# tangjiapeng/DiffuScene

Measured on AMD Instinct MI355X. Metric: denoiser steps/sec (train + 1000-step sample) at B=256, N=80 objects, higher is better.
Workload: dtype f32 (operands split 3xbf16, 6 products, f32 accumulate); 1 GPU; uncond living/dining rooms (config/uncond/diffusion_livingrooms_instancond_lat32_v.yaml scaled to N=80), B=256 scenes per GPU, N=80, C=65, T=1000, mode=both; global_batch=256, parallelism=single

## Files before the change

### diffuscene_amd/_lib.py

```python
import ctypes as C
import os

_HERE = os.path.dirname(os.path.abspath(__file__))
LIB_PATH = os.path.join(_HERE, "libdiffuscene_hip.so")
if os.environ.get("DSC_HIP_LIB"):
    LIB_PATH = os.path.abspath(os.environ["DSC_HIP_LIB"])

ACT_NONE, ACT_GELU, ACT_SILU, ACT_LEAKY01 = 0, 1, 2, 3
SS_NONE, SS_PER_TOKEN, SS_PER_SCENE, SS_PER_SLOT, SS_BY_INDEX = 0, 1, 2, 3, 4
MEAN_EPS, MEAN_X0, MEAN_V = 0, 1, 2
TILE_GN_80_W8, TILE_GN_80_W4, TILE_160x256, TILE_160x128_W4 = 1, 2, 5, 8
TILE_WAVE_GN, TILE_WAVE_DENSE, TILE_WAVE_GN_64 = 10, 11, 12
F32_TILE_160x256, F32_TILE_160x128, F32_TILE_128x128, F32_TILE_96x128, F32_TILE_64x64 = 0, 1, 2, 3, 4
DSC_PLANES_NONE = -100
GEMM_ROW_INVARIANT = 1
WS_MAX = 64
MAX_TOKENS_PER_SCENE = 160
STATS_MAX_OBJECTS, STATS_ONE_WAVE_MAX = 160, 32

_ERR = {-1: "DSC_EINVAL (bad shape / null pointer)", -2: "DSC_EALIGN (16-byte alignment required)",
        -3: "DSC_ERANGE (size outside kernel limits)"}

c_f32p = C.c_void_p
c_i64p = C.c_void_p
# ... 118 lines not shown
    "dsc_gather_max_bwd_f32": (C.c_int, [c_f32p, C.c_int64, C.c_void_p, C.c_void_p, C.c_int32, C.c_int32, C.c_int32, c_f32p,
                                         C.c_int64, C.c_void_p]),
    "dsc_bn_workspace_floats": (C.c_int64, [C.c_int64, C.c_int32]),
    "dsc_batchnorm_fwd_f32": (C.c_int, [c_f32p, C.c_int64, c_f32p, c_f32p, C.c_int64, C.c_int32, C.c_float, C.c_float,
                                        C.c_int32, c_f32p, c_f32p, c_f32p, c_f32p, c_f32p, c_f32p, c_f32p, C.c_int64,
                                        C.c_void_p]),
    "dsc_batchnorm_eval_f32": (C.c_int, [c_f32p, C.c_int64, c_f32p, c_f32p, c_f32p, c_f32p, C.c_int64, C.c_int32, C.c_int32,
                                         c_f32p, C.c_void_p]),
    "dsc_batchnorm_bwd_f32": (C.c_int, [c_f32p, c_f32p, c_f32p, c_f32p, c_f32p, C.c_int64, C.c_int32, C.c_int32, c_f32p,
                                        c_f32p, c_f32p, c_f32p, C.c_int64, C.c_void_p]),
    "dsc_rowmax_f32": (C.c_int, [c_f32p, C.c_int64, C.c_int32, C.c_int32, C.c_int32, c_f32p, C.c_void_p, C.c_void_p]),
    "dsc_rowmax_bwd_f32": (C.c_int, [c_f32p, C.c_void_p, C.c_int32, C.c_int32, C.c_int32, c_f32p, C.c_void_p]),
    "dsc_point_affine_f32": (C.c_int, [c_f32p, C.c_int64, C.c_int32, c_f32p, C.c_int64, c_f32p, C.c_int32, C.c_int32,
                                       C.c_int32, C.c_int32, c_f32p, C.c_void_p]),
    "dsc_point_affine_bwd_f32": (C.c_int, [c_f32p, c_f32p, C.c_int64, C.c_int32, c_f32p, C.c_int64, C.c_int32, C.c_int32,
                                           C.c_int32, C.c_int32, c_f32p, C.c_int64, c_f32p, C.c_int64, c_f32p, c_f32p,
                                           C.c_int64, C.c_void_p]),
    "dsc_postfilter_compact_f32": (C.c_int, [c_f32p, C.c_int32, C.c_int32, C.c_int32, C.c_int32, C.c_int32, C.c_int32, c_f32p,
                                             C.c_void_p, C.c_void_p]),
    "dsc_gemm_tn_f32": (C.c_int, [c_f32p, C.c_int64, C.c_int32, c_f32p, C.c_int64, C.c_int32, c_f32p, C.c_int64, c_f32p,
                                  C.c_int64, c_f32p, C.c_int32, C.c_int32, C.c_int32, c_f32p, C.c_int64, C.c_void_p]),
    "dsc_gemm_tn_workspace_floats": (C.c_int64, [C.c_int32, C.c_int32, C.c_int32]),
    "dsc_gemm_tn_grouped_f32": (C.c_int, [C.c_void_p, C.c_int32, C.c_int32, C.c_int32, c_f32p, C.c_int64, C.c_int64,
                                          C.c_void_p]),
    "dsc_gemm_tn_grouped_split_f32": (C.c_int, [C.c_void_p, C.c_int32, C.c_int32, C.c_void_p, C.c_int32, C.c_int32, c_f32p, C.c_int64,
                                                C.c_int64, C.c_int32, C.c_void_p]),
    "dsc_set_tn_split_form": (C.c_int, [C.c_int32]),
    "dsc_get_tn_split_form": (C.c_int, []),
    "dsc_colsum_f32": (C.c_int, [c_f32p, C.c_int64, C.c_int32, C.c_int32, c_f32p, c_f32p, C.c_int64, C.c_void_p]),
    "dsc_colsum_grouped_f32": (C.c_int, [C.c_void_p, C.c_int32, C.c_int32, C.c_void_p]),
    "dsc_gn_silu_bwd_f32": (C.c_int, [c_f32p, C.c_int64, c_f32p, C.c_int64, c_f32p, c_f32p, c_f32p, C.c_int64, C.c_int32,
                                      c_f32p, C.c_int64, c_f32p, c_f32p, c_f32p, C.c_int64, c_f32p, C.c_int64, C.c_int32,
                                      C.c_int32, C.c_int32, C.c_float, C.c_void_p]),
    "dsc_weight_standardize_bwd_f32": (C.c_int, [C.POINTER(WsBwdItem), C.c_int32, C.c_float, C.c_void_p]),
    "dsc_layernorm_bwd_f32": (C.c_int, [c_f32p, C.c_int64, c_f32p, c_f32p, C.c_int64, c_f32p, C.c_int64, c_f32p, C.c_int64, c_f32p,
                                        C.c_int32, C.c_int32, C.c_int32, C.c_float, C.c_void_p]),
    "dsc_linear_attention_bwd_f32": (C.c_int, [c_f32p, C.c_int64] * 7 + [C.c_int32, C.c_int32, C.c_int32, C.c_float,
                                                                          C.c_void_p]),
    "dsc_attention_bwd_f32": (C.c_int, [c_f32p, C.c_int64] * 7 + [C.c_int32, C.c_int32, C.c_float, C.c_void_p]),
    "dsc_retrieve_nearest_f32": (C.c_int, [c_f32p, C.c_void_p, C.c_void_p, c_f32p, C.c_void_p, C.c_void_p, C.c_int32,
                                           C.c_int32, C.c_int32, C.c_void_p, c_f32p, C.c_void_p]),
    "dsc_box_bounds_f32": (C.c_int, [c_f32p, c_f32p, c_f32p, C.c_void_p, C.c_int32, C.c_int32, c_f32p, C.c_void_p]),
    "dsc_scene_stats_f32": (C.c_int, [c_f32p, c_f32p, C.c_void_p, C.c_void_p, C.c_int32, C.c_int32, C.c_int32, C.c_int32,
                                      C.c_void_p, C.c_void_p, C.c_void_p, C.c_void_p, C.c_void_p, C.c_void_p, c_f32p, C.c_void_p]),
    "dsc_encode_scene_batch_f32": (C.c_int, [c_i64p, c_f32p, c_f32p, c_f32p, c_f32p, c_f32p, C.c_int32, C.c_int32, c_i64p,
                                             C.c_void_p, C.c_void_p, C.c_void_p, C.c_int32, C.POINTER(C.c_double), c_f32p,
                                             C.c_int64, c_i64p, C.c_int32, C.c_int32, C.c_void_p]),
    "dsc_chamfer3d_forward_f32": (C.c_int, [c_f32p, c_f32p, c_f32p, c_f32p, C.c_void_p, C.c_void_p, C.c_int32, C.c_int32,
                                            C.c_int32, C.c_void_p]),
    "dsc_chamfer3d_backward_f32": (C.c_int, [c_f32p, c_f32p, c_f32p, c_f32p, C.c_void_p, C.c_void_p, c_f32p, c_f32p,
                                             C.c_int32, C.c_int32, C.c_int32, C.c_void_p]),
    "dsc_grad_sumsq_f32": (C.c_int, [C.c_void_p, C.c_int32, C.c_void_p, C.c_void_p]),
    "dsc_clip_coef_f32": (C.c_int, [C.c_void_p, C.c_int32, C.c_float, c_f32p, c_f32p, C.c_void_p]),
    "dsc_adam_step_f32": (C.c_int, [C.c_void_p, C.c_int32, C.c_float, C.c_float, C.c_float, C.c_float, C.c_float, C.c_float,
                                    c_f32p, C.c_void_p]),
    "dsc_ddpm_loss_f32": (C.c_int, [c_f32p, c_f32p, c_f32p, c_i64p, c_f32p, c_f32p, c_f32p, c_f32p, C.POINTER(C.c_float),
                                    c_f32p, c_f32p, c_f32p] + [C.c_int32] * 12 + [C.c_float, C.c_int32, C.c_void_p]),
    "dsc_copy2d_f32": (C.c_int, [c_f32p, C.c_int64, c_f32p, C.c_int64, C.c_int32, C.c_int32, C.c_void_p]),
    "dsc_add2d_f32": (C.c_int, [c_f32p, C.c_int64, c_f32p, C.c_int64, C.c_int32, C.c_int32, C.c_void_p]),
    "dsc_activation_bwd_f32": (C.c_int, [c_f32p, c_f32p, c_f32p, C.c_int64, C.c_int32, C.c_void_p]),
    "dsc_transpose_batched_f32": (C.c_int, [C.POINTER(WsItem), C.c_int32, C.c_void_p]),
    "dsc_transpose_f32": (C.c_int, [c_f32p, C.c_int64, c_f32p, C.c_int64, C.c_int32, C.c_int32, C.c_void_p]),
    "dsc_complete_overwrite_f32": (C.c_int, [c_f32p, c_f32p, c_f32p, c_i64p, c_f32p, c_f32p, C.c_int32, C.c_int32,
                                             C.c_int32, C.c_int32, C.c_int32, C.c_void_p]),
    "dsc_complete_overwrite_ragged_f32": (C.c_int, [c_f32p, c_f32p, c_f32p, c_i64p, c_i64p, c_f32p, c_f32p, C.c_int32, C.c_int32,
                                                    C.c_int32, C.c_int32, C.c_int32, C.c_void_p]),
# ... 103 lines not shown
```

### diffuscene_amd/csrc/train.hip

```cpp
#define DSC_BAD_INDEX_COUNTER
#include "dsc_common.h"

namespace {

constexpr int TN_BK = 32;
constexpr int TN_LD = 132;

struct TnArgs {
    const float* a1; long lda1; int k1;
    const float* a2; long lda2; int k2;
    const float* dy; long ldd;
    float* out; long ldo;
    float* bias_out;
    long slab;
    long bias_slab;
    int m, n, kvalid;
    int chunk;
    int ktiles;
};

__device__ __forceinline__ void tn_block(const TnArgs& p, const int it, const int jt, const int split, float* As, float* Bs) {
    const int tid = threadIdx.x, lane = tid & 63, wave = tid >> 6;
    const int wi = wave >> 1, wj = wave & 1;
    const int l31 = lane & 31, half = lane >> 5;
    const int i0 = it * 128, j0 = jt * 128;
    const long m_begin = (long)split * p.chunk;
    const long m_end = (m_begin + p.chunk < p.m) ? m_begin + p.chunk : p.m;

    const float* ab;
    long lda;
    int ic;
    int kseg;
    if (i0 < p.k1) { ab = p.a1; lda = p.lda1; ic = i0; kseg = p.k1; }
    else           { ab = p.a2; lda = p.lda2; ic = i0 - p.k1; kseg = p.k2; }
// ... 427 lines not shown
    const int c = blockIdx.x * 64 + (threadIdx.x & 63);
    if (blockIdx.x * 64 >= it.n) return;
    const int rq = threadIdx.x >> 6;
    float s = 0.f;
    if (c < it.n) {
        const float* xp = it.x + (long)rq * it.ldx + c;
        const long step = 4 * it.ldx;
        int r = rq;
        float s0 = 0.f, s1 = 0.f, s2 = 0.f, s3 = 0.f;
        for (; r + 28 < it.m; r += 32, xp += 8 * step) {
            const float v0 = xp[0], v1 = xp[step], v2 = xp[2 * step], v3 = xp[3 * step];
            const float v4 = xp[4 * step], v5 = xp[5 * step], v6 = xp[6 * step], v7 = xp[7 * step];
            s0 += v0; s1 += v1; s2 += v2; s3 += v3;
            s0 += v4; s1 += v5; s2 += v6; s3 += v7;
        }
        for (; r < it.m; r += 4, xp += step) s0 += xp[0];
        s = (s0 + s1) + (s2 + s3);
    }
    red[rq][threadIdx.x & 63] = s;
    __syncthreads();
    if (rq == 0 && c < it.n) it.out[c] = (red[0][threadIdx.x] + red[1][threadIdx.x]) + (red[2][threadIdx.x] + red[3][threadIdx.x]);
}

struct GnBwdArgs {
    const float* z; long ldz;
    const float* dy; long ldy;
    const float* gamma; const float* beta;
    const float* ss; long ld_ss; int ss_mode;
    float* dz; long lddz;
    float* dgamma_p; float* dbeta_p; float* dbias_p;
    long pstride;
    float* dss; long ld_dss;
    int n_tok, C; float eps;
};

__device__ __forceinline__ float block_sum(float v, float* red) {
    v = wave_sum(v);
    __syncthreads();
    if ((threadIdx.x & 63) == 0) red[threadIdx.x >> 6] = v;
    __syncthreads();
    return (red[0] + red[1]) + (red[2] + red[3]);
}

__global__ __launch_bounds__(256) void gn_silu_bwd_kernel(const GnBwdArgs p) {
    extern __shared__ float gnb_cache[];
    __shared__ float red[4];
    __shared__ float csum[5][4][64];
    const int b = blockIdx.x >> 3, g = blockIdx.x & 7;
    const int cl = threadIdx.x & 63, tq = threadIdx.x >> 6;
    const int c = g * 64 + cl;
    const int N = p.n_tok;
    const long tok0 = (long)b * N;
    const float inv_cnt = 1.0f / (64.0f * (float)N);
    float* zc = gnb_cache + cl;
    float* dc = gnb_cache + (long)N * 64 + cl;
    float s = 0.f;
    {
        const float* zp = p.z + (tok0 + tq) * p.ldz + c;
        const float* dp = p.dy + (tok0 + tq) * p.ldy + c;
        const long zs = 4 * p.ldz, ds = 4 * p.ldy;
#pragma unroll 5
        for (int j = tq; j < N; j += 4) {
            const float zv = *zp, dv = *dp;
            zp += zs; dp += ds;
            zc[j * 64] = zv; dc[j * 64] = dv;
            s += zv;
// ... 150 lines not shown
    const float m2 = bsum(S2) * inv_cnt;
#pragma unroll
    for (int i = 0; i < NIT; ++i) {
        const int j = tr + 16 * i;
        if (j < N) {
            f32x4 dzv;
#pragma unroll
            for (int e = 0; e < 4; ++e) { dzv[e] = rs * (dv[i][e] - m1 - zv[i][e] * m2); Gz[e] += dzv[e]; }
            *reinterpret_cast<f32x4*>(p.dz + (tok0 + j) * p.lddz + c) = dzv;
        }
    }
    auto fold = [&](f32x4 v, int slot) {
#pragma unroll
        for (int e = 0; e < 4; ++e) {
            float t = v[e];
            t += __shfl_xor(t, 16, 64);
            t += __shfl_xor(t, 32, 64);
            if ((threadIdx.x & 63) < 16) csum[slot][wave][cq * 4 + e] = t;
        }
    };
    fold(Gg, 0); fold(Gb, 1); fold(Gz, 2); fold(Gsc, 3); fold(Gsh, 4);
    __syncthreads();
    if (threadIdx.x < 64) {
        const int cl = threadIdx.x;
        const long o = (long)b * p.pstride + g * 64 + cl;
        p.dgamma_p[o] = (csum[0][0][cl] + csum[0][1][cl]) + (csum[0][2][cl] + csum[0][3][cl]);
        p.dbeta_p[o] = (csum[1][0][cl] + csum[1][1][cl]) + (csum[1][2][cl] + csum[1][3][cl]);
        p.dbias_p[o] = (csum[2][0][cl] + csum[2][1][cl]) + (csum[2][2][cl] + csum[2][3][cl]);
        if (p.dss && p.ss_mode == DSC_SS_PER_SCENE) {
            p.dss[(long)b * p.ld_dss + g * 64 + cl] = (csum[3][0][cl] + csum[3][1][cl]) + (csum[3][2][cl] + csum[3][3][cl]);
            p.dss[(long)b * p.ld_dss + p.C + g * 64 + cl] = (csum[4][0][cl] + csum[4][1][cl]) + (csum[4][2][cl] + csum[4][3][cl]);
        }
    }
}

struct WsBwdItem { const float* w; const float* dwh; float* dw; int rows; int cols; };
struct WsBwdBatch { WsBwdItem it[DSC_WS_MAX]; };

__global__ __launch_bounds__(256) void ws_bwd_kernel(const WsBwdBatch bch, const float eps) {
    __shared__ float red[4];
    const WsBwdItem it = bch.it[blockIdx.y];
    const int row = blockIdx.x;
    if (row >= it.rows) return;
    const float* w = it.w + (long)row * it.cols;
    const float* g = it.dwh + (long)row * it.cols;
    float* o = it.dw + (long)row * it.cols;
    constexpr int MAXE = 8;
    float v[MAXE], gv[MAXE];
    float s = 0.f;
#pragma unroll
    for (int i = 0; i < MAXE; ++i) {
        const int c = threadIdx.x + 256 * i;
        v[i] = (c < it.cols) ? w[c] : 0.f;
        gv[i] = (c < it.cols) ? g[c] : 0.f;
        s += v[i];
    }
    const float inv = 1.0f / (float)it.cols;
    const float mean = block_sum(s, red) * inv;
    float s2 = 0.f;
#pragma unroll
    for (int i = 0; i < MAXE; ++i) {
        const int c = threadIdx.x + 256 * i;
        const float d = (c < it.cols) ? v[i] - mean : 0.f;
        s2 += d * d;
    }
    const float rs = 1.0f / sqrtf(block_sum(s2, red) * inv + eps);
// ... 675 lines not shown
                                   int64_t partial_stride, float* dss, int64_t ld_dss, int32_t scenes,
                                   int32_t tokens_per_scene, int32_t channels, float eps, dsc_stream_t stream) {
    if (!z || !dy || !gamma || !beta || !dz || !dgamma_p || !dbeta_p || !dbias_p) return DSC_EINVAL;
    if (scenes < 1 || tokens_per_scene < 1 || channels != 512) return DSC_ERANGE;
    if (ss_mode != DSC_SS_NONE && !scale_shift) return DSC_EINVAL;
    GnBwdArgs p{z, (long)ldz, dy, (long)ldy, gamma, beta, ss_mode != DSC_SS_NONE ? scale_shift : nullptr, (long)ld_ss,
                ss_mode, dz, (long)lddz, dgamma_p, dbeta_p, dbias_p, (long)partial_stride, dss, (long)ld_dss, tokens_per_scene,
                channels, eps};
    if (tokens_per_scene > 160) return DSC_ERANGE;
    const size_t lds = (size_t)2 * tokens_per_scene * 64 * sizeof(float);
    DSC_CLEAR_STALE_ERROR();
    const bool v4 = ((ldz | ldy | lddz) & 3) == 0 && dsc_aligned16(z) && dsc_aligned16(dy) && dsc_aligned16(dz) &&
                    dsc_aligned16(gamma) && dsc_aligned16(beta) &&
                    (!p.ss || (dsc_aligned16(p.ss) && (ld_ss & 3) == 0)) &&
                    (!dss || (dsc_aligned16(dss) && (ld_dss & 3) == 0));
    if (lds > 48 * 1024) {
        static bool raised = false;
        if (!raised) {
            hipError_t e = hipFuncSetAttribute(reinterpret_cast<const void*>(gn_silu_bwd_kernel),
                                               hipFuncAttributeMaxDynamicSharedMemorySize, 96 * 1024);
            if (e != hipSuccess) return (int)e;
            raised = true;
        }
    }
    hipStream_t hs = static_cast<hipStream_t>(stream);
    if (v4 && tokens_per_scene <= 32)
        hipLaunchKernelGGL(gn_silu_bwd_reg_kernel<2>, dim3(scenes * 8), dim3(256), 0, hs, p);
    else if (v4 && tokens_per_scene <= 80)
        hipLaunchKernelGGL(gn_silu_bwd_reg_kernel<5>, dim3(scenes * 8), dim3(256), 0, hs, p);
    else if (v4)
        hipLaunchKernelGGL(gn_silu_bwd_reg_kernel<10>, dim3(scenes * 8), dim3(256), 0, hs, p);
    else
        hipLaunchKernelGGL(gn_silu_bwd_kernel, dim3(scenes * 8), dim3(256), lds, static_cast<hipStream_t>(stream), p);
    DSC_LAUNCH_CHECK();
    return 0;
}

extern "C" int dsc_weight_standardize_bwd_f32(const dsc_ws_bwd_item* items, int32_t count, float eps, dsc_stream_t stream) {
    if (!items || count < 1 || count > DSC_WS_MAX) return DSC_EINVAL;
    WsBwdBatch b;
    int maxrows = 0;
    for (int i = 0; i < count; ++i) {
        if (!items[i].w || !items[i].dw_std || !items[i].dw || items[i].rows < 1 || items[i].cols < 1) return DSC_EINVAL;
        if (items[i].cols > 2048) return DSC_ERANGE;
        b.it[i] = WsBwdItem{items[i].w, items[i].dw_std, items[i].dw, items[i].rows, items[i].cols};
        if (items[i].rows > maxrows) maxrows = items[i].rows;
    }
    DSC_CLEAR_STALE_ERROR();
    hipLaunchKernelGGL(ws_bwd_kernel, dim3(maxrows, count), dim3(256), 0, static_cast<hipStream_t>(stream), b, eps);
    DSC_LAUNCH_CHECK();
    return 0;
}

extern "C" int dsc_layernorm_bwd_f32(const float* x, int64_t ldx, const float* g, const float* dy, int64_t ldy, float* dx,
                                     int64_t lddx, const float* addend, int64_t ldadd, float* dg_partial, int32_t partial_rows,
                                     int32_t m, int32_t d, float eps, dsc_stream_t stream) {
    if (!x || !g || !dy || !dx || !dg_partial || m < 1 || partial_rows < 1) return DSC_EINVAL;
    if (d != 512) return DSC_ERANGE;
    if (!dsc_aligned16(x) || !dsc_aligned16(g) || !dsc_aligned16(dy) || !dsc_aligned16(dx) || (ldx & 3) || (ldy & 3) ||
        (lddx & 3) || (addend && (!dsc_aligned16(addend) || (ldadd & 3)))) return DSC_EALIGN;
    DSC_CLEAR_STALE_ERROR();
    hipLaunchKernelGGL(layernorm_bwd_kernel, dim3(partial_rows), dim3(256), 0, static_cast<hipStream_t>(stream),
                       x, (long)ldx, g, dy, (long)ldy, dx, (long)lddx, addend, (long)ldadd, dg_partial, m, eps);
    DSC_LAUNCH_CHECK();
    return 0;
}
// ... 390 lines not shown
```

### diffuscene_amd/ops.py

```python
import ctypes as C
import numbers

import torch

from . import _lib
from ._lib import (ACT_GELU, ACT_NONE, ACT_SILU, MEAN_EPS, MEAN_V, MEAN_X0, SS_NONE, SS_PER_SCENE,
                   SS_PER_SLOT, SS_PER_TOKEN, GemmArgs, SplitItem, WsItem)


def stream_ptr():
    return torch.cuda.current_stream().cuda_stream


def _dev(t, name="tensor", dtype=torch.float32):
    if not isinstance(t, torch.Tensor) or not t.is_cuda:
        raise RuntimeError("diffuscene_amd: %s must live on a HIP device (no CPU fallback exists)" % name)
    if t.dtype != dtype:
        raise RuntimeError("diffuscene_amd: %s must be %s, got %s" % (name, dtype, t.dtype))
    return t


def issue(rec, stream=None):
    name, args, _ = rec
    _lib.check(_lib.fn(name)(*args, stream if stream is not None else stream_ptr()), name)
# ... 850 lines not shown
def colsum(x, out=None):
    if out is None:
        out = torch.empty((x.shape[1],), device=x.device, dtype=torch.float32)
    ws = scratch(x.device, 64 * x.shape[1])
    issue(colsum_rec(x, out, ws.data_ptr(), ws.numel()))
    return out


def device_table(arr, device):
    import numpy as np
    return torch.from_numpy(np.frombuffer(bytes(arr), dtype=np.uint8).copy()).to(device)


def colsum_grouped_rec(pairs, device):
    arr = (_lib.ColsumItem * len(pairs))()
    for i, (x, out) in enumerate(pairs):
        if not (out.is_contiguous() and out.numel() == x.shape[1]):
            raise RuntimeError("colsum_grouped: out must be a contiguous (%d,) tensor" % x.shape[1])
        arr[i].x, arr[i].ldx = _mat(x, "x")
        arr[i].m, arr[i].n, arr[i].out = x.shape[0], x.shape[1], out.data_ptr()
    table = device_table(arr, device)
    return "dsc_colsum_grouped_f32", (table.data_ptr(), len(pairs), max(x.shape[1] for x, _ in pairs)), (table, pairs)


def gn_silu_bwd_rec(z, dy, gamma, beta, ss, ss_mode, dz, part, order, dss, scenes, n_tok, eps=1e-5):
    zp, ldz, dp, ldy, sp, ld_ss, dzp, lddz, dsp, ld_dss = _mats((z, "z"), (dy, "dy"), (ss, "ss"), (dz, "dz"), (dss, "dss"))
    Cc = z.shape[1]
    pg, pb, pB = (_mat(part, "part")[0] + 4 * Cc * o for o in order)
    return ("dsc_gn_silu_bwd_f32", (zp, ldz, dp, ldy, _dev(gamma).data_ptr(), _dev(beta).data_ptr(), sp, ld_ss,
                                    ss_mode if sp else SS_NONE, dzp, lddz, pg, pb, pB, part.stride(0), dsp, ld_dss, scenes, n_tok,
                                    Cc, eps), (z, dy, gamma, beta, ss, dz, part, dss))


def gn_silu_bwd(z, dy, gamma, beta, ss, ss_mode, scenes, n_tok, eps=1e-5):
    M, Cc = z.shape
    dz = torch.empty((M, Cc), device=z.device, dtype=torch.float32)
    part = torch.empty((scenes, 3 * Cc), device=z.device, dtype=torch.float32)
    dss = None
    if ss is not None and ss_mode != SS_NONE:
        dss = torch.empty((scenes if ss_mode == SS_PER_SCENE else M, 2 * Cc), device=z.device, dtype=torch.float32)
    issue(gn_silu_bwd_rec(z, dy, gamma, beta, ss if dss is not None else None, ss_mode, dz, part, (0, 1, 2), dss, scenes, n_tok, eps))
    red = colsum(part)
    return dz, red[:Cc], red[Cc:2 * Cc], red[2 * Cc:], dss


def weight_standardize_bwd_rec(triples, eps=1e-5):
    arr = (_lib.WsBwdItem * len(triples))()
    for j, (w, g, o) in enumerate(triples):
        w2, g2, o2 = as2d(_dev(w)), _dev(g), as2d(_dev(o))
        if not (w2.is_contiguous() and g2.is_contiguous() and o2.is_contiguous()):
            raise RuntimeError("weight_standardize_bwd needs contiguous matrices")
        arr[j].w, arr[j].dw_std, arr[j].dw = w2.data_ptr(), g2.data_ptr(), o2.data_ptr()
        arr[j].rows, arr[j].cols = w2.shape
    return "dsc_weight_standardize_bwd_f32", (arr, len(triples), eps), (arr, triples)


def weight_standardize_bwd(weights, dw_stds, eps=1e-5):
    outs = [torch.empty_like(as2d(w)) for w in weights]
    for i in range(0, len(weights), _lib.WS_MAX):
        s = slice(i, i + _lib.WS_MAX)
        issue(weight_standardize_bwd_rec(list(zip(weights[s], dw_stds[s], outs[s])), eps))
    return outs


def layernorm_bwd_rec(x, g, dy, dx, dg_part, addend=None, eps=1e-5):
    run = _mats((dy, "dy"), (dx, "dx"), (addend, "addend"))
# ... 66 lines not shown
```

### diffuscene_amd/train_plan.py

```python
import ctypes as C
import os

import torch

from . import engine, ops
from ._lib import ACT_GELU, ACT_NONE, ACT_SILU, SS_NONE, SS_PER_SCENE, SS_PER_SLOT, SS_PER_TOKEN

D = 512
HID = 128


def _as2d(w):
    return w.view(w.shape[0], w.shape[1]) if w.dim() == 3 else w


class H:
    __slots__ = ("t", "g", "ng", "act_of", "g_pre", "uses", "gn_of", "gn_part")

    def __init__(self, t, needs_grad=True):
        self.t, self.g, self.ng = t, None, needs_grad
        self.uses = 0
        self.act_of = None
        self.g_pre = None
        self.gn_of = None
# ... 243 lines not shown
                        raise RuntimeError("gemm_tn_grouped: split outputs must be dense [n][kvalid]")
                    g.ws_offset = ws_off
                    ws_off += (g.n * g.kvalid + g.n) * splits
            return ws_off
        if use_split:
            tile_k = 256 if (self.lib.fn("dsc_get_tn_split_form")() == 2
                             and all(not (it.get("a2") is not None and it["a"].shape[1] % 256) for it in items)) else 128
            rounds = int(os.environ.get("DSC_TN_ROUNDS", "3" if tile_k == 128 else "2"))
            splits, _ = tn_token_slices(shapes, 256, rounds * 256 - (64 if tile_k == 256 else 0), tile_k)
            ws_off = slab_offsets(splits)
            table = ops.device_table(arr, self.device)
            bmap = np.asarray(tn_block_map(shapes, tile_k=tile_k), dtype=np.int32).reshape(-1, 2)
            want_tiles = sum(((n + 255) // 256) * ((k + tile_k - 1) // tile_k) for _, n, k in shapes)
            assert int((bmap[:, 0] >= 0).sum()) == want_tiles, "block map must cover every 256 x %d tile exactly once" % tile_k
            bmap_dev = torch.from_numpy(bmap.copy()).to(self.device)
            return self._with_scratch(ws_off, lambda wp, wn: self._call(
                "dsc_gemm_tn_grouped_split_f32", table.data_ptr(), len(items), total, bmap_dev.data_ptr(), bmap.shape[0], splits,
                wp if splits > 1 else None, wn if splits > 1 else 0, ws_off, tile_k, keep=(table, items, bmap_dev)))
        splits, _ = tn_token_slices(shapes, 128, 8 * 512)
        ws_off = slab_offsets(splits)
        table = ops.device_table(arr, self.device)
        return self._with_scratch(ws_off, lambda wp, wn: self._call(
            "dsc_gemm_tn_grouped_f32", table.data_ptr(), len(items), total, splits, wp if splits > 1 else None,
            wn if splits > 1 else 0, ws_off, keep=(table, items)))

    def colsum(self, x, out):
        return self._with_scratch(64 * x.shape[1], lambda wp, wn: self._rec(ops.colsum_rec(x, out, wp, wn)))

    def colsum_grouped(self, pairs):
        return self._rec(ops.colsum_grouped_rec(pairs, self.device))

    def gn_bwd(self, z, dy, gamma, beta, ss, ss_mode, dz, part, dss, scenes, n_tok):
        return self._rec(ops.gn_silu_bwd_rec(z, dy, gamma, beta, ss, ss_mode, dz, part, (1, 2, 0), dss, scenes, n_tok))

    def ws_bwd(self, weights, dws, outs):
        n = self.lib.WS_MAX
        return [self._rec(ops.weight_standardize_bwd_rec(list(zip(weights[i:i + n], dws[i:i + n], outs[i:i + n]))))
                for i in range(0, len(weights), n)]

    def layernorm_bwd(self, x, g, dy, dx, dg_part, addend=None):
        return self._rec(ops.layernorm_bwd_rec(x, g, dy, dx, dg_part, addend))

    def linattn_bwd(self, q, k, v, dout, dq, dk, dv, scenes, nq, nk, scale):
        return self._rec(ops.linear_attention_bwd_rec(q, k, v, dout, dq, dk, dv, scenes, nq, nk, scale))

    def attn_bwd(self, q, k, v, dout, dq, dk, dv, scenes, n, scale):
        return self._rec(ops.attention_bwd_rec(q, k, v, dout, dq, dk, dv, scenes, n, scale))

    def act_bwd(self, x, dy, dx, kind):
        return self._rec(ops.activation_bwd_rec(x, dy, dx, kind))

    def transpose_many(self, pairs):
        batch = [(w, o) for w, o in pairs if w.is_contiguous() and o.is_contiguous()]
        steps = [self._rec(ops.transpose_rec(w, o)) for w, o in pairs if not (w.is_contiguous() and o.is_contiguous())]
        n = self.lib.WS_MAX
        return steps + [self._rec(ops.transpose_batched_rec(batch[i:i + n])) for i in range(0, len(batch), n)]

    def copy(self, dst, src):
        return self._rec(ops.copy2d_rec(dst, src))

    def add(self, dst, src):
        return self._rec(ops.add2d_rec(dst, src))


    def run(self, steps, stream):
        check = self.lib.check
# ... 336 lines not shown
            if not dy.is_contiguous():
                d = self.new(*dy.shape)
                self.emit(self.be.copy(d, dy))
                dy = d
            self.g_write(x, lambda dst: self.emit(self.be.act_bwd(x.t, dy, dst, kind)))
        self._tape.append(bw)
        return y

    def conv_gn(self, a, blk, a2=None, ss=None, ss_mode=SS_NONE, dss=None, residual=None):
        conv, norm = blk.proj, blk.norm
        w_std = self.ws_std[id(conv)]
        rows = a.t.shape[0]
        y, z = H(self.new(rows, D)), self.new(rows, D)
        self._use(a, a2, residual)
        self.emit(self.be.gemm_gn(a.t, w_std, y.t, conv.bias, norm.weight, norm.bias, self.N, a2.t if a2 is not None else None,
                                  ss, ss_mode, residual.t if residual is not None else None, z))

        if residual is None:
            y.gn_of = dict(z=z, gamma=norm.weight, beta=norm.bias, ss=ss, ss_mode=ss_mode if ss is not None else SS_NONE,
                           dss=dss if (ss is not None and ss_mode == SS_PER_SCENE) else None, n_tok=self.N)

        def bw():
            dy = y.g
            if dy is None and y.g_pre is None:
                return
            scenes = rows // self.N
            slot_tmp = None
            if y.g_pre is not None:
                dz, part = y.g_pre, y.gn_part
            else:
                dz = self.new(rows, D)
                part = self.new(scenes, 3 * D)
                dss_arg = dss
                if ss is not None and ss_mode == SS_PER_SLOT:
                    slot_tmp = self.new(rows, 2 * D)
                    dss_arg = slot_tmp
                self.emit(self.be.gn_bwd(z, dy, norm.weight, norm.bias, ss, ss_mode, dz, part, dss_arg, scenes, self.N))
            o_b, o_g, o_be = (self.flat.grad_range(p)[0] for p in (conv.bias, norm.weight, norm.bias))
            if o_g == o_b + D and o_be == o_g + D:
                self.colsum_later(part, self.flat.G[o_b:o_b + 3 * D], params=(conv.bias, norm.weight, norm.bias))
            else:
                tmp = self.new(1, 3 * D)

                def scatter(tmp=tmp):
                    for i, p in enumerate((conv.bias, norm.weight, norm.bias)):
                        self.emit(self.be.copy(self.flat.grad_view(p).view(1, D), tmp[:, i * D:(i + 1) * D]))
                self.colsum_later(part, tmp.view(-1), params=(conv.bias, norm.weight, norm.bias), after=scatter)
            if slot_tmp is not None:
                red = self.new(self.N, 2 * D)
                self.emit(self.be.colsum(slot_tmp.view(scenes, self.N * 2 * D), red.view(-1)))
                self.emit(self.be.copy(dss, red))
            self.g_gemm(a, a2, dz, self.ws_t[id(conv)])
            self.tn(a.t, dz, self.dws[id(conv)], a2.t if a2 is not None else None)
            self._ws_pending.append(conv)
            if residual is not None:
                self.g_alias(residual, dy)
        self._tape.append(bw)
        return y

    def resblock(self, rb, a, a2, ss_pair, post=None):
        if post is not None:
            self._tape.append(post)
        ss, mode, dss = ss_pair
        h = self.conv_gn(a, rb.block1, a2=a2, ss=ss, ss_mode=mode, dss=dss)
        r = self.linear(a, rb.res_conv.weight, rb.res_conv.bias, a2=a2) if rb.has_res_conv else a
        return self.conv_gn(h, rb.block2, residual=r)

    def layernorm(self, x, gain, residual=None):
        g = gain.view(-1)
        y = H(self.new(*x.t.shape))
# ... 347 lines not shown
```

### include/diffuscene_hip.h

```cpp
#ifndef DIFFUSCENE_HIP_H
#define DIFFUSCENE_HIP_H

#include <stdint.h>

#ifdef __cplusplus
extern "C" {
#endif

typedef void* dsc_stream_t;

#define DSC_EINVAL   (-1)
#define DSC_EALIGN   (-2)
#define DSC_ERANGE   (-3)

#define DSC_ACT_NONE 0
#define DSC_ACT_GELU 1
#define DSC_ACT_SILU 2
#define DSC_ACT_LEAKY01 3

#define DSC_SS_NONE      0
#define DSC_SS_PER_TOKEN 1
#define DSC_SS_PER_SCENE 2
#define DSC_SS_PER_SLOT  3
#define DSC_SS_BY_INDEX  4
// ... 226 lines not shown
int64_t dsc_gemm_tn_workspace_floats(int32_t m, int32_t n, int32_t k);

typedef struct dsc_tn_group {
    const float* a1; int64_t lda1; int32_t k1;
    const float* a2; int64_t lda2; int32_t k2;
    const float* dy; int64_t ldd;
    float* out; int64_t ldo;
    float* dbias;
    int32_t m, n, kvalid;
    int32_t tile0;
    int64_t ws_offset;
    int32_t tile0s;
} dsc_tn_group;
int dsc_gemm_tn_grouped_f32(const dsc_tn_group* groups_dev, int32_t count, int32_t total_tiles, int32_t splits,
                            float* workspace, int64_t workspace_floats, int64_t workspace_needed, dsc_stream_t stream);
int dsc_gemm_tn_grouped_split_f32(const dsc_tn_group* groups_dev, int32_t count, int32_t total_tiles, const int32_t* block_map_dev,
                                  int32_t blocks, int32_t splits, float* workspace, int64_t workspace_floats, int64_t workspace_needed,
                                  int32_t tile_k, dsc_stream_t stream);

int dsc_set_tn_split_form(int32_t form);
int dsc_get_tn_split_form(void);

int dsc_colsum_f32(const float* x, int64_t ldx, int32_t m, int32_t n, float* out, float* workspace,
                   int64_t workspace_floats, dsc_stream_t stream);

typedef struct dsc_colsum_item { const float* x; int64_t ldx; int32_t m, n; float* out; } dsc_colsum_item;
int dsc_colsum_grouped_f32(const dsc_colsum_item* items_dev, int32_t count, int32_t max_n, dsc_stream_t stream);

int dsc_gn_silu_bwd_f32(const float* z, int64_t ldz, const float* dy, int64_t ldy, const float* gamma,
                        const float* beta, const float* scale_shift, int64_t ld_ss, int32_t ss_mode,
                        float* dz, int64_t lddz, float* dgamma_p, float* dbeta_p, float* dbias_p, int64_t partial_stride,
                        float* dss, int64_t ld_dss, int32_t scenes, int32_t tokens_per_scene, int32_t channels,
                        float eps, dsc_stream_t stream);

typedef struct dsc_ws_bwd_item { const float* w; const float* dw_std; float* dw; int32_t rows; int32_t cols; } dsc_ws_bwd_item;
int dsc_weight_standardize_bwd_f32(const dsc_ws_bwd_item* items, int32_t count, float eps, dsc_stream_t stream);

int dsc_layernorm_bwd_f32(const float* x, int64_t ldx, const float* g, const float* dy, int64_t ldy, float* dx,
                          int64_t lddx, const float* addend, int64_t ldadd, float* dg_partial, int32_t partial_rows, int32_t m,
                          int32_t d, float eps, dsc_stream_t stream);

int dsc_linear_attention_bwd_f32(const float* q, int64_t ldq, const float* k, int64_t ldk, const float* v, int64_t ldv,
                                 const float* dout, int64_t ldo, float* dq, int64_t lddq, float* dk, int64_t lddk,
                                 float* dv, int64_t lddv, int32_t scenes, int32_t nq, int32_t nk, float scale,
                                 dsc_stream_t stream);

int dsc_attention_bwd_f32(const float* q, int64_t ldq, const float* k, int64_t ldk, const float* v, int64_t ldv,
                          const float* dout, int64_t ldo, float* dq, int64_t lddq, float* dk, int64_t lddk,
                          float* dv, int64_t lddv, int32_t scenes, int32_t n, float scale, dsc_stream_t stream);

int dsc_ddpm_loss_f32(const float* target, const float* out, const float* x_t, const int64_t* t,
                      const float* loss_weight, const float* ca, const float* cb, const float* alphas_cumprod,
                      const float* bounds, float* losses, float* parts, float* dout, int32_t b, int32_t n, int32_t c,
                      int32_t translation_dim, int32_t size_dim, int32_t bbox_dim, int32_t class_dim,
                      int32_t objectness_dim, int32_t objfeat_dim, int32_t loss_separate, int32_t loss_iou,
                      int32_t mean_type, float grad_scale, int32_t num_timesteps, dsc_stream_t stream);

int dsc_copy2d_f32(float* dst, int64_t ldd, const float* src, int64_t lds, int32_t rows, int32_t cols, dsc_stream_t stream);
int dsc_add2d_f32(float* dst, int64_t ldd, const float* src, int64_t lds, int32_t rows, int32_t cols, dsc_stream_t stream);

int dsc_activation_bwd_f32(const float* x, const float* dy, float* dx, int64_t count, int32_t act, dsc_stream_t stream);

int dsc_transpose_f32(const float* in, int64_t ldi, float* out, int64_t ldo, int32_t rows, int32_t cols,
                      dsc_stream_t stream);
int dsc_transpose_batched_f32(const dsc_ws_item* items, int32_t count, dsc_stream_t stream);

// ... 74 lines not shown
```

Baseline: 62.20 steps/s.

## Accumulate per-slot scale/shift grads over scene strips in GN-SiLU backward

Adds a strip-based GroupNorm+SiLU backward kernel for per-slot scale/shift mode. Each block handles several scenes, keeps the per-slot dscale/dshift sums in registers and prefetches the next scene's inputs. A small reduction kernel then sums the strip partials. Before, a full rows x 2D temporary was written and column-summed over all scenes. This cuts that temporary's memory traffic and the colsum pass, at the cost of fewer blocks (less parallelism) and an extra launch.

```diff
diff --git a/diffuscene_amd/_lib.py b/diffuscene_amd/_lib.py
--- a/diffuscene_amd/_lib.py
+++ b/diffuscene_amd/_lib.py
@@ -174,6 +174,11 @@
     "dsc_gn_silu_bwd_f32": (C.c_int, [c_f32p, C.c_int64, c_f32p, C.c_int64, c_f32p, c_f32p, c_f32p, C.c_int64, C.c_int32,
                                       c_f32p, C.c_int64, c_f32p, c_f32p, c_f32p, C.c_int64, c_f32p, C.c_int64, C.c_int32,
                                       C.c_int32, C.c_int32, C.c_float, C.c_void_p]),
+    "dsc_gn_bwd_strip_len": (C.c_int, [C.c_int32]),
+    "dsc_gn_silu_bwd_strips_f32": (C.c_int, [c_f32p, C.c_int64, c_f32p, C.c_int64, c_f32p, c_f32p, c_f32p, C.c_int64, c_f32p, C.c_int64,
+                                             c_f32p, c_f32p, c_f32p, C.c_int64, c_f32p, C.c_int32, C.c_int32, C.c_int32, C.c_int32,
+                                             C.c_int32, C.c_float, C.c_void_p]),
+    "dsc_gn_slot_reduce_f32": (C.c_int, [c_f32p, C.c_int32, C.c_int32, C.c_int32, c_f32p, C.c_int64, C.c_void_p]),
     "dsc_weight_standardize_bwd_f32": (C.c_int, [C.POINTER(WsBwdItem), C.c_int32, C.c_float, C.c_void_p]),
     "dsc_layernorm_bwd_f32": (C.c_int, [c_f32p, C.c_int64, c_f32p, c_f32p, C.c_int64, c_f32p, C.c_int64, c_f32p, C.c_int64, c_f32p,
                                         C.c_int32, C.c_int32, C.c_int32, C.c_float, C.c_void_p]),
diff --git a/diffuscene_amd/csrc/train.hip b/diffuscene_amd/csrc/train.hip
--- a/diffuscene_amd/csrc/train.hip
+++ b/diffuscene_amd/csrc/train.hip
@@ -1,5 +1,6 @@
 #define DSC_BAD_INDEX_COUNTER
 #include "dsc_common.h"
+#include <cstdlib>
 
 namespace {
 
@@ -493,6 +494,8 @@
     long pstride;
     float* dss; long ld_dss;
     int n_tok, C; float eps;
+    int scenes, strip;
+    float* slot_part;
 };
 
 __device__ __forceinline__ float block_sum(float v, float* red) {
@@ -709,6 +712,162 @@
             p.dss[(long)b * p.ld_dss + p.C + g * 64 + cl] = (csum[4][0][cl] + csum[4][1][cl]) + (csum[4][2][cl] + csum[4][3][cl]);
         }
     }
+}
+
+template <int NIT>
+__global__ __launch_bounds__(256) void gn_silu_bwd_slot_kernel(const GnBwdArgs p) {
+    __shared__ float red[2][4];
+    __shared__ float csum[3][4][64];
+    const int strip = blockIdx.x >> 3, g = blockIdx.x & 7;
+    const int cq = threadIdx.x & 15, tr = threadIdx.x >> 4;
+    const int wave = threadIdx.x >> 6;
+    const int c = g * 64 + cq * 4;
+    const int N = p.n_tok;
+    const float inv_cnt = 1.0f / (64.0f * (float)N);
+    const int b0 = strip * p.strip;
+    const int b1 = b0 + p.strip < p.scenes ? b0 + p.strip : p.scenes;
+    const f32x4 ga = *reinterpret_cast<const f32x4*>(p.gamma + c);
+    const f32x4 be = *reinterpret_cast<const f32x4*>(p.beta + c);
+    f32x4 zv[NIT], dv[NIT], zn[NIT], dn[NIT];
+    f32x4 s1r[NIT], shr[NIT];
+    f32x4 Asc[NIT], Ash[NIT];
+    auto bsum = [&](float v, int slot) {
+        v = wave_sum(v);
+        float* r = red[slot];
+        if ((threadIdx.x & 63) == 0) r[wave] = v;
+        __syncthreads();
+        return (r[0] + r[1]) + (r[2] + r[3]);
+    };
+    auto fetch = [&](int b, f32x4 (&zr)[NIT], f32x4 (&dr)[NIT]) {
+        const long tok0 = (long)b * N;
+#pragma unroll
+        for (int i = 0; i < NIT; ++i) {
+            const int j = tr + 16 * i;
+            const long row = tok0 + (j < N ? j : 0);
+            zr[i] = *reinterpret_cast<const f32x4*>(p.z + row * p.ldz + c);
+            dr[i] = *reinterpret_cast<const f32x4*>(p.dy + row * p.ldy + c);
+        }
+    };
+    auto scene = [&](const int b) {
+        const long tok0 = (long)b * N;
+        float s = 0.f;
+#pragma unroll
+        for (int i = 0; i < NIT; ++i) {
+            if (tr + 16 * i >= N) { zv[i] = f32x4{0.f, 0.f, 0.f, 0.f}; dv[i] = zv[i]; }
+            s += (zv[i][0] + zv[i][1]) + (zv[i][2] + zv[i][3]);
+        }
+        const float mu = bsum(s, 0) * inv_cnt;
+        s = 0.f;
+#pragma unroll
+        for (int i = 0; i < NIT; ++i)
+            if (tr + 16 * i < N) {
+#pragma unroll
+                for (int e = 0; e < 4; ++e) { const float d = zv[i][e] - mu; s += d * d; }
+            }
+        const float rs = 1.0f / sqrtf(bsum(s, 1) * inv_cnt + p.eps);
+        float S1 = 0.f, S2 = 0.f;
+        f32x4 Gg = {0.f, 0.f, 0.f, 0.f}, Gb = Gg, Gz = Gg;
+#pragma unroll
+        for (int i = 0; i < NIT; ++i) {
+            if (tr + 16 * i < N) {
+                f32x4 xh, dxh;
+#pragma unroll
+                for (int e = 0; e < 4; ++e) {
+                    xh[e] = (zv[i][e] - mu) * rs;
+                    const float gh = ga[e] * xh[e] + be[e];
+                    const float u = gh * s1r[i][e] + shr[i][e];
+                    const float sig = __builtin_amdgcn_rcpf(1.0f + __expf(-u));
+                    const float du = dv[i][e] * (sig * (1.0f + u * (1.0f - sig)));
+                    const float dgh = du * s1r[i][e];
+                    dxh[e] = dgh * ga[e];
+                    S1 += dxh[e]; S2 += dxh[e] * xh[e];
+                    Gg[e] += dgh * xh[e]; Gb[e] += dgh;
+                    Asc[i][e] += du * gh; Ash[i][e] += du;
+                }
+                zv[i] = xh;
+                dv[i] = dxh;
+            }
+        }
+        const float m1 = bsum(S1, 0) * inv_cnt;
+        const float m2 = bsum(S2, 1) * inv_cnt;
+#pragma unroll
+        for (int i = 0; i < NIT; ++i) {
+            const int j = tr + 16 * i;
+            if (j < N) {
+                f32x4 dzv;
+#pragma unroll
+                for (int e = 0; e < 4; ++e) { dzv[e] = rs * (dv[i][e] - m1 - zv[i][e] * m2); Gz[e] += dzv[e]; }
+                *reinterpret_cast<f32x4*>(p.dz + (tok0 + j) * p.lddz + c) = dzv;
+            }
+        }
+        auto fold = [&](f32x4 v, int slot) {
+#pragma unroll
+            for (int e = 0; e < 4; ++e) {
+                float t = v[e];
+                t += __shfl_xor(t, 16, 64);
+                t += __shfl_xor(t, 32, 64);
+                if ((threadIdx.x & 63) < 16) csum[slot][wave][cq * 4 + e] = t;
+            }
+        };
+        fold(Gg, 0); fold(Gb, 1); fold(Gz, 2);
+        __syncthreads();
+        if (threadIdx.x < 64) {
+            const int cl = threadIdx.x;
+            const long o = (long)b * p.pstride + g * 64 + cl;
+            p.dgamma_p[o] = (csum[0][0][cl] + csum[0][1][cl]) + (csum[0][2][cl] + csum[0][3][cl]);
+            p.dbeta_p[o] = (csum[1][0][cl] + csum[1][1][cl]) + (csum[1][2][cl] + csum[1][3][cl]);
+            p.dbias_p[o] = (csum[2][0][cl] + csum[2][1][cl]) + (csum[2][2][cl] + csum[2][3][cl]);
+        }
+    };
+#pragma unroll
+    for (int i = 0; i < NIT; ++i) {
+        const int j = tr + 16 * i;
+        const float* sr = p.ss + (long)(j < N ? j : 0) * p.ld_ss;
+        const f32x4 a = *reinterpret_cast<const f32x4*>(sr + c);
+        shr[i] = *reinterpret_cast<const f32x4*>(sr + p.C + c);
+#pragma unroll
+        for (int e = 0; e < 4; ++e) s1r[i][e] = 1.0f + a[e];
+        Asc[i] = f32x4{0.f, 0.f, 0.f, 0.f};
+        Ash[i] = Asc[i];
+    }
+    fetch(b0, zv, dv);
+    int b = b0;
+    for (; b + 1 < b1; ++b) {
+        fetch(b + 1, zn, dn);
+        scene(b);
+#pragma unroll
+        for (int i = 0; i < NIT; ++i) { zv[i] = zn[i]; dv[i] = dn[i]; }
+    }
+    scene(b);
+    float* o = p.slot_part + (long)strip * N * (2 * p.C);
+#pragma unroll
+    for (int i = 0; i < NIT; ++i) {
+        const int j = tr + 16 * i;
+        if (j < N) {
+            *reinterpret_cast<f32x4*>(o + (long)j * (2 * p.C) + c) = Asc[i];
+            *reinterpret_cast<f32x4*>(o + (long)j * (2 * p.C) + p.C + c) = Ash[i];
+        }
+    }
+}
+
+__global__ __launch_bounds__(256) void gn_slot_reduce_kernel(const float* __restrict__ part, int strips, int n_tok, int cols,
+                                                            float* __restrict__ out, long ldo) {
+    __shared__ float red[4][64];
+    const int col = blockIdx.x * 64 + (threadIdx.x & 63);
+    const int rq = threadIdx.x >> 6;
+    const int j = blockIdx.y;
+    float s0 = 0.f, s1 = 0.f;
+    if (col < cols) {
+        const long step = (long)n_tok * cols;
+        const float* xp = part + ((long)rq * n_tok + j) * cols + col;
+        int r = rq;
+        for (; r + 4 < strips; r += 8, xp += 8 * step) { s0 += xp[0]; s1 += xp[4 * step]; }
+        if (r < strips) s0 += xp[0];
+    }
+    red[rq][threadIdx.x & 63] = s0 + s1;
+    __syncthreads();
+    if (rq == 0 && col < cols)
+        out[(long)j * ldo + col] = (red[0][threadIdx.x] + red[1][threadIdx.x]) + (red[2][threadIdx.x] + red[3][threadIdx.x]);
 }
 
 struct WsBwdItem { const float* w; const float* dwh; float* dw; int rows; int cols; };
@@ -1450,6 +1609,53 @@
         hipLaunchKernelGGL(gn_silu_bwd_reg_kernel<10>, dim3(scenes * 8), dim3(256), 0, hs, p);
     else
         hipLaunchKernelGGL(gn_silu_bwd_kernel, dim3(scenes * 8), dim3(256), lds, static_cast<hipStream_t>(stream), p);
+    DSC_LAUNCH_CHECK();
+    return 0;
+}
+
+extern "C" int dsc_gn_bwd_strip_len(int32_t scenes) {
+    static const int forced = [] { const char* e = getenv("DSC_GN_STRIP"); const int v = e ? atoi(e) : 0; return v >= 1 && v <= 64 ? v : 0; }();
+    if (scenes < 1) return 0;
+    if (forced) return forced;
+    for (int s = 8; s > 1; s >>= 1)
+        if ((scenes + s - 1) / s >= 32) return s;
+    return 1;
+}
+
+extern "C" int dsc_gn_silu_bwd_strips_f32(const float* z, int64_t ldz, const float* dy, int64_t ldy, const float* gamma,
+                                          const float* beta, const float* scale_shift, int64_t ld_ss, float* dz, int64_t lddz,
+                                          float* dgamma_p, float* dbeta_p, float* dbias_p, int64_t partial_stride,
+                                          float* slot_partials, int32_t strips, int32_t strip_len, int32_t scenes,
+                                          int32_t tokens_per_scene, int32_t channels, float eps, dsc_stream_t stream) {
+    if (!z || !dy || !gamma || !beta || !scale_shift || !dz || !dgamma_p || !dbeta_p || !dbias_p || !slot_partials) return DSC_EINVAL;
+    if (scenes < 1 || tokens_per_scene < 1 || tokens_per_scene > 160 || channels != 512) return DSC_ERANGE;
+    if (strip_len < 1 || strips != (scenes + strip_len - 1) / strip_len) return DSC_EINVAL;
+    GnBwdArgs p{z, (long)ldz, dy, (long)ldy, gamma, beta, scale_shift, (long)ld_ss, DSC_SS_PER_SLOT, dz, (long)lddz, dgamma_p, dbeta_p,
+                dbias_p, (long)partial_stride, nullptr, 0, tokens_per_scene, channels, eps, scenes, strip_len, slot_partials};
+    if (((ldz | ldy | lddz | ld_ss) & 3) != 0 || !dsc_aligned16(z) || !dsc_aligned16(dy) || !dsc_aligned16(dz) || !dsc_aligned16(gamma) ||
+        !dsc_aligned16(beta) || !dsc_aligned16(scale_shift) || !dsc_aligned16(slot_partials))
+        return DSC_EALIGN;
+    DSC_CLEAR_STALE_ERROR();
+    hipStream_t hs = static_cast<hipStream_t>(stream);
+    const dim3 grid(strips * 8);
+    if (tokens_per_scene <= 32)
+        hipLaunchKernelGGL(gn_silu_bwd_slot_kernel<2>, grid, dim3(256), 0, hs, p);
+    else if (tokens_per_scene <= 80)
+        hipLaunchKernelGGL(gn_silu_bwd_slot_kernel<5>, grid, dim3(256), 0, hs, p);
+    else
+        hipLaunchKernelGGL(gn_silu_bwd_slot_kernel<10>, grid, dim3(256), 0, hs, p);
+    DSC_LAUNCH_CHECK();
+    return 0;
+}
+
+extern "C" int dsc_gn_slot_reduce_f32(const float* slot_partials, int32_t strips, int32_t tokens_per_scene, int32_t cols, float* out,
+                                      int64_t ldo, dsc_stream_t stream) {
+    if (!slot_partials || !out) return DSC_EINVAL;
+    if (strips < 1 || tokens_per_scene < 1 || tokens_per_scene > 65535 || cols < 1) return DSC_ERANGE;
+    if (ldo < cols) return DSC_EINVAL;
+    DSC_CLEAR_STALE_ERROR();
+    hipLaunchKernelGGL(gn_slot_reduce_kernel, dim3((cols + 63) / 64, tokens_per_scene), dim3(256), 0, static_cast<hipStream_t>(stream),
+                       slot_partials, strips, tokens_per_scene, cols, out, (long)ldo);
     DSC_LAUNCH_CHECK();
     return 0;
 }
diff --git a/diffuscene_amd/ops.py b/diffuscene_amd/ops.py
--- a/diffuscene_amd/ops.py
+++ b/diffuscene_amd/ops.py
@@ -906,6 +906,34 @@
                                     Cc, eps), (z, dy, gamma, beta, ss, dz, part, dss))
 
 
+def gn_strip_len(scenes):
+    return int(_lib.fn("dsc_gn_bwd_strip_len")(scenes))
+
+
+def gn_strips_aligned(*tensors):
+    return all(t.data_ptr() % 16 == 0 and (t.dim() < 2 or t.shape[0] == 1 or t.stride(0) % 4 == 0) for t in tensors)
+
+
+def gn_silu_bwd_strips_rec(z, dy, gamma, beta, ss, dz, part, order, slot_part, strip_len, scenes, n_tok, eps=1e-5):
+    zp, ldz, dp, ldy, sp, ld_ss, dzp, lddz = _mats((z, "z"), (dy, "dy"), (ss, "ss"), (dz, "dz"))
+    Cc = z.shape[1]
+    strips = (scenes + strip_len - 1) // strip_len
+    if not (slot_part.is_contiguous() and slot_part.numel() == strips * n_tok * 2 * Cc):
+        raise RuntimeError("gn_silu_bwd_strips: slot_part must be a contiguous tensor of %d x %d x %d floats" % (strips, n_tok, 2 * Cc))
+    pg, pb, pB = (_mat(part, "part")[0] + 4 * Cc * o for o in order)
+    return ("dsc_gn_silu_bwd_strips_f32", (zp, ldz, dp, ldy, _dev(gamma).data_ptr(), _dev(beta).data_ptr(), sp, ld_ss, dzp, lddz,
+                                           pg, pb, pB, part.stride(0), _dev(slot_part).data_ptr(), strips, strip_len, scenes, n_tok,
+                                           Cc, eps), (z, dy, gamma, beta, ss, dz, part, slot_part))
+
+
+def gn_slot_reduce_rec(slot_part, out, n_tok):
+    op, ldo = _mat(out, "out")
+    cols = out.shape[1]
+    if not (slot_part.dim() == 2 and slot_part.is_contiguous() and slot_part.shape[1] == n_tok * cols and out.shape[0] == n_tok):
+        raise RuntimeError("gn_slot_reduce: slot_part must be contiguous [strips, %d * %d], out [%d, %d]" % (n_tok, cols, n_tok, cols))
+    return "dsc_gn_slot_reduce_f32", (_dev(slot_part).data_ptr(), slot_part.shape[0], n_tok, cols, op, ldo), (slot_part, out)
+
+
 def gn_silu_bwd(z, dy, gamma, beta, ss, ss_mode, scenes, n_tok, eps=1e-5):
     M, Cc = z.shape
     dz = torch.empty((M, Cc), device=z.device, dtype=torch.float32)
diff --git a/diffuscene_amd/train_plan.py b/diffuscene_amd/train_plan.py
--- a/diffuscene_amd/train_plan.py
+++ b/diffuscene_amd/train_plan.py
@@ -299,6 +299,14 @@
 
     def gn_bwd(self, z, dy, gamma, beta, ss, ss_mode, dz, part, dss, scenes, n_tok):
         return self._rec(ops.gn_silu_bwd_rec(z, dy, gamma, beta, ss, ss_mode, dz, part, (1, 2, 0), dss, scenes, n_tok))
+
+    def gn_bwd_slot(self, z, dy, gamma, beta, ss, dz, part, dss, scenes, n_tok, new):
+        if n_tok > 160 or not ops.gn_strips_aligned(z, dy, ss, dz, gamma, beta):
+            return None
+        strip = ops.gn_strip_len(scenes)
+        slot_part = new((scenes + strip - 1) // strip, n_tok * dss.shape[1])
+        return [self._rec(ops.gn_silu_bwd_strips_rec(z, dy, gamma, beta, ss, dz, part, (1, 2, 0), slot_part, strip, scenes, n_tok)),
+                self._rec(ops.gn_slot_reduce_rec(slot_part, dss, n_tok))]
 
     def ws_bwd(self, weights, dws, outs):
         n = self.lib.WS_MAX
@@ -701,10 +709,16 @@
                 dz = self.new(rows, D)
                 part = self.new(scenes, 3 * D)
                 dss_arg = dss
+                steps = None
                 if ss is not None and ss_mode == SS_PER_SLOT:
-                    slot_tmp = self.new(rows, 2 * D)
-                    dss_arg = slot_tmp
-                self.emit(self.be.gn_bwd(z, dy, norm.weight, norm.bias, ss, ss_mode, dz, part, dss_arg, scenes, self.N))
+                    if hasattr(self.be, "gn_bwd_slot"):
+                        steps = self.be.gn_bwd_slot(z, dy, norm.weight, norm.bias, ss, dz, part, dss, scenes, self.N, self.new)
+                    if steps is None:
+                        slot_tmp = self.new(rows, 2 * D)
+                        dss_arg = slot_tmp
+                if steps is None:
+                    steps = self.be.gn_bwd(z, dy, norm.weight, norm.bias, ss, ss_mode, dz, part, dss_arg, scenes, self.N)
+                self.emit(steps)
             o_b, o_g, o_be = (self.flat.grad_range(p)[0] for p in (conv.bias, norm.weight, norm.bias))
             if o_g == o_b + D and o_be == o_g + D:
                 self.colsum_later(part, self.flat.G[o_b:o_b + 3 * D], params=(conv.bias, norm.weight, norm.bias))
diff --git a/include/diffuscene_hip.h b/include/diffuscene_hip.h
--- a/include/diffuscene_hip.h
+++ b/include/diffuscene_hip.h
@@ -282,6 +282,15 @@
                         float* dz, int64_t lddz, float* dgamma_p, float* dbeta_p, float* dbias_p, int64_t partial_stride,
                         float* dss, int64_t ld_dss, int32_t scenes, int32_t tokens_per_scene, int32_t channels,
                         float eps, dsc_stream_t stream);
+
+int dsc_gn_bwd_strip_len(int32_t scenes);
+int dsc_gn_silu_bwd_strips_f32(const float* z, int64_t ldz, const float* dy, int64_t ldy, const float* gamma,
+                               const float* beta, const float* scale_shift, int64_t ld_ss, float* dz, int64_t lddz,
+                               float* dgamma_p, float* dbeta_p, float* dbias_p, int64_t partial_stride, float* slot_partials,
+                               int32_t strips, int32_t strip_len, int32_t scenes, int32_t tokens_per_scene, int32_t channels,
+                               float eps, dsc_stream_t stream);
+int dsc_gn_slot_reduce_f32(const float* slot_partials, int32_t strips, int32_t tokens_per_scene, int32_t cols, float* out,
+                           int64_t ldo, dsc_stream_t stream);
 
 typedef struct dsc_ws_bwd_item { const float* w; const float* dw_std; float* dw; int32_t rows; int32_t cols; } dsc_ws_bwd_item;
 int dsc_weight_standardize_bwd_f32(const dsc_ws_bwd_item* items, int32_t count, float eps, dsc_stream_t stream);
```

New measurement: 62.65 steps/s (median of 6 runs). About the same (+0.7%).
